# linum-uqam/ViT-OCM-WMSegmentation

Measured on AMD Instinct MI355X. Metric: OCM tiles/s (224x224, ViT-S/16 attention-map inference), higher is better.
Workload: dtype bf16x3

## Files before the change

vit-ocm-wmsegmentation_amd/csrc/engine.hip:

```cpp
#include <stdarg.h>
#include <stdio.h>
#include <string.h>

#include <atomic>
#include <mutex>
#include <string>
#include <vector>

#include "host_common.h"
#include "launch.h"
#include "attn_plan.h"
#include "otsu.h"

static thread_local std::string g_err;

int ocm_fail(int code, const char *fmt, ...) {
    char buf[512];
    va_list ap;
    va_start(ap, fmt);
    vsnprintf(buf, sizeof buf, fmt, ap);
    va_end(ap);
    g_err = buf;
    return code;
}
// ... 272 lines not shown
    void *xn;
    void *q, *k;
    void *vt;
    void *ctx;
    void *hid;
    float *lse;
    float *qkv32;
    float *kpart;
    size_t kpart_bytes;
    float *part;
    float *stats;
    float *shift;
    float *tok_shift;
    size_t bytes;
};

static Workspace carve(const ocm_vit *h, int batch, int n, char *base) {
    Workspace w;
    size_t off = 0;
    auto take = [&](size_t bytes) {
        char *pch = base ? base + off : nullptr;
        off += (bytes + 255) & ~(size_t)255;
        return pch;
    };
    const size_t T = (size_t)batch * n, BH = (size_t)batch * h->H, np = ocm_n_pad_for(h->prec, n);
    const size_t e = h->esz;
    w.x = (float *)take(T * h->D * 4);
    w.xn = take(T * h->D * e);
    w.lse = (float *)take(BH * n * 4);
    w.stats = h->can_fold() ? (float *)take(2 * T * (size_t)(h->D / 64) * 8) : nullptr;
    w.shift = h->can_fold() ? (float *)take(2 * T * 4) : nullptr;
    w.tok_shift = h->can_fold() ? (float *)take((size_t)n * 4) : nullptr;
    w.part = (h->prec == 2 && T <= (size_t)OCM_SPLITK_MAX_ROWS) ? (float *)take((size_t)OCM_SPLITK * T * h->D * 4) : nullptr;
    w.kpart_bytes = attention_ksplit_bytes(h->prec, batch, n, h->H, h->hd);
    w.kpart = w.kpart_bytes ? (float *)take(w.kpart_bytes) : nullptr;
    const size_t base_off = off;
    w.q = w.k = w.vt = nullptr;
    w.qkv32 = nullptr;
    if (h->mfma_heads()) {
        w.q = take(BH * np * h->hd * e);
        w.k = take(BH * np * h->hd * e);
        w.vt = take(BH * np * h->hd * e);
    } else {
        w.qkv32 = (float *)take(3 * T * h->D * 4);
    }
    w.ctx = take(T * h->D * e);
    const size_t attn_end = off;
    off = base_off;
    w.hid = take(T * h->M * e);
    if (off < attn_end) off = attn_end;
    w.bytes = off;
    return w;
}

extern "C" size_t ocm_vit_workspace_bytes(const ocm_vit_t *h, int32_t batch, int32_t n_tokens) {
    if (!h || batch <= 0 || n_tokens <= 1) return 0;
    return carve(h, batch, n_tokens, nullptr).bytes;
}

static int check_ws(const ocm_vit *h, int batch, int n, void *ws, size_t ws_bytes) {
    if (!ws) return fail(OCM_ENOMEM, "workspace is null");
    if ((uintptr_t)ws & 255) return fail(OCM_EINVAL, "workspace must be 256-byte aligned");
    const size_t need = carve(h, batch, n, nullptr).bytes;
    if (ws_bytes < need) return fail(OCM_ENOMEM, "workspace too small: %zu < %zu bytes", ws_bytes, need);
    return OCM_OK;
}

static int run_attention(const ocm_vit *h, const Workspace &w, int batch, int n, bool attn_only, float *out_attn, float *out_qkv,
                         const int32_t *query_rows, int n_rows, float *out_rows, const char *qkv_w, const float *qkv_b,
                         const LnFold &ln, hipStream_t s) {
    const int H = h->H, np = ocm_n_pad_for(h->prec, n), pc = h->prec;
    const float scale = h->cfg.qk_scale;
    const bool want_v = !(attn_only && !out_qkv);
    if (!h->mfma_heads()) {
        float *qkv = out_qkv ? out_qkv : w.qkv32;
        { PROF(OCM_K_QKV, s); HIP_TRY(launch_qkv(pc, w.xn, qkv_w, qkv_b, nullptr, nullptr, nullptr, qkv, batch, n, np, H, h->hd, want_v, s, ln)); }
        { PROF(OCM_K_ATTN, s); HIP_TRY(launch_attention_generic(pc, qkv, attn_only ? nullptr : w.ctx, out_attn, query_rows, n_rows, out_rows, batch, n, H, h->hd, scale, s)); }
        return OCM_OK;
    }
    void *vt_dst = want_v ? w.vt : nullptr;
    { PROF(OCM_K_QKV, s); HIP_TRY(launch_qkv(pc, w.xn, qkv_w, qkv_b, w.q, w.k, vt_dst, out_qkv, batch, n, np, H, h->hd, want_v, s, ln)); }
    if (out_rows && !out_attn) { PROF(OCM_K_PROBS, s); HIP_TRY(launch_attention_rows(pc, w.q, w.k, query_rows, n_rows, out_rows, batch, n, np, H, scale, s, h->hd)); }
    if (attn_only && !out_attn) return OCM_OK;
    { PROF(OCM_K_ATTN, s); HIP_TRY(launch_attention(pc, w.q, w.k, w.vt, attn_only ? nullptr : w.ctx, out_attn ? w.lse : nullptr, batch, n, np, H, scale, s, h->hd, w.kpart, w.kpart_bytes)); }
    if (out_attn) {
        PROF(OCM_K_PROBS, s);
        HIP_TRY(launch_attention_probs(pc, w.q, w.k, w.lse, out_attn, batch, n, np, H, scale, s, h->hd, query_rows, n_rows, out_rows));
    }
    return OCM_OK;
}

static int run_block(const ocm_vit *h, int i, const Workspace &w, float *x, int batch, int n, bool attn_only,
                     float *out_attn, float *out_qkv, const int32_t *query_rows, int n_rows, float *out_rows,
                     hipStream_t s, bool xn_ready = false, const float *next_g = nullptr, const float *next_b = nullptr,
                     bool *xn_out = nullptr) {
    const BlockP &bp = h->blk[i];
    const int D = h->D, T = batch * n;
    const float eps = h->cfg.ln_eps;
    const int pc = h->prec, lnk = ln_kind_of_prec(pc);
    const long t128 = (long)((T + 127) / 128) * (D / 128);
    const int fuse_opt = h->opt[OCM_OPT_FUSE_LN];
    const bool fuse_ln = linear_resid_ln_supported(D) && fuse_opt != 1 && ((T >= 8192 && t128 < 512) || fuse_opt == 2);
    if (xn_out) *xn_out = false;
    if (!xn_ready) { PROF(OCM_K_LN, s); HIP_TRY(launch_layernorm(x, h->ptr<float>(bp.ln1_g), h->ptr<float>(bp.ln1_b), w.xn, lnk, T, D, eps, s)); }
    if (int rc = run_attention(h, w, batch, n, attn_only, out_attn, out_qkv, query_rows, n_rows, out_rows, h->ptr<char>(bp.qkv_w),
                               h->ptr<float>(bp.qkv_b), LnFold(), s))
        return rc;
    if (attn_only) return OCM_OK;
    if (fuse_ln) {
        PROF(OCM_K_PROJ, s);
        HIP_TRY(launch_linear_resid_ln(pc, w.ctx, h->ptr<char>(bp.proj_w), h->ptr<float>(bp.proj_b), x, x, h->ptr<float>(bp.ln2_g), h->ptr<float>(bp.ln2_b), w.xn, T, D, D, eps, s));
    } else {
        { PROF(OCM_K_PROJ, s); HIP_TRY(launch_linear(pc, w.ctx, h->ptr<char>(bp.proj_w), h->ptr<float>(bp.proj_b), x, x, T, D, D, OCM_EPI_BIAS_RESID_F32, s)); }
        { PROF(OCM_K_LN, s); HIP_TRY(launch_layernorm(x, h->ptr<float>(bp.ln2_g), h->ptr<float>(bp.ln2_b), w.xn, lnk, T, D, eps, s)); }
    }
    { PROF(OCM_K_FC1, s); HIP_TRY(launch_linear(pc, w.xn, h->ptr<char>(bp.fc1_w), h->ptr<float>(bp.fc1_b), nullptr, w.hid, T, h->M, D, OCM_EPI_BIAS_GELU_BF16, s)); }
    if (fuse_ln && next_g && next_b) {
        PROF(OCM_K_FC2, s);
        HIP_TRY(launch_linear_resid_ln(pc, w.hid, h->ptr<char>(bp.fc2_w), h->ptr<float>(bp.fc2_b), x, x, next_g, next_b, w.xn, T, D, h->M, eps, s));
        if (xn_out) *xn_out = true;
    } else {
        PROF(OCM_K_FC2, s);
        StatsOut so;
        if (fuse_opt == 0) so.part = w.part;
        HIP_TRY(launch_linear(pc, w.hid, h->ptr<char>(bp.fc2_w), h->ptr<float>(bp.fc2_b), x, x, T, D, h->M, OCM_EPI_BIAS_RESID_F32, s, LnFold(), so));
    }
    return OCM_OK;
}

static int run_block_folded(const ocm_vit *h, int i, const Workspace &w, float *x, int batch, int n, bool attn_only,
                            float *out_attn, float *out_qkv, const int32_t *query_rows, int n_rows, float *out_rows,
                            hipStream_t s) {
    const BlockP &bp = h->blk[i];
    const int D = h->D, T = batch * n, pc = h->prec;
    float *st_in = w.stats, *st_mid = w.stats + (size_t)T * (D / 64) * 2, *st_out = w.stats;
    LnFold ln1, ln2;
    ln1.stats = st_in, ln1.c = h->ptr<float>(bp.qkv_c), ln1.d = h->ptr<float>(bp.qkv_d), ln1.inv_dim = 1.0f / D, ln1.eps = h->cfg.ln_eps;
    ln2.stats = st_mid, ln2.c = h->ptr<float>(bp.fc1_c), ln2.d = h->ptr<float>(bp.fc1_d), ln2.inv_dim = 1.0f / D, ln2.eps = h->cfg.ln_eps;
    ln1.nslot = ln2.nslot = D / 64;
    if (int rc = run_attention(h, w, batch, n, attn_only, out_attn, out_qkv, query_rows, n_rows, out_rows, h->ptr<char>(bp.qkv_wf),
                               nullptr, ln1, s))
        return rc;
    if (attn_only) return OCM_OK;
    StatsOut so_mid, so_out;
    so_mid.xs = w.xn, so_mid.stats = st_mid;
    so_out.xs = w.xn, so_out.stats = st_out;
    float *sh_in = w.shift, *sh_mid = w.shift + T;
    so_mid.shift = sh_mid, so_mid.prev_stats = st_in, so_mid.prev_shift = sh_in;
    so_out.shift = sh_in, so_out.prev_stats = st_mid, so_out.prev_shift = sh_mid;
    so_out.part = w.part;
    { PROF(OCM_K_PROJ, s); HIP_TRY(launch_linear(pc, w.ctx, h->ptr<char>(bp.proj_w), h->ptr<float>(bp.proj_b), x, x, T, D, D, OCM_EPI_BIAS_RESID_F32, s, LnFold(), so_mid)); }
    { PROF(OCM_K_FC1, s); HIP_TRY(launch_linear(pc, w.xn, h->ptr<char>(bp.fc1_wf), nullptr, nullptr, w.hid, T, h->M, D, OCM_EPI_BIAS_GELU_BF16, s, ln2)); }
    { PROF(OCM_K_FC2, s); HIP_TRY(launch_linear(pc, w.hid, h->ptr<char>(bp.fc2_w), h->ptr<float>(bp.fc2_b), x, x, T, D, h->M, OCM_EPI_BIAS_RESID_F32, s, LnFold(), so_out)); }
    return OCM_OK;
}

static int check_tiles(const ocm_vit *h, const ocm_vit_io *io, int *n_out) {
    if (!io) return fail(OCM_EINVAL, "io is null");
    if (!io->image) return fail(OCM_EINVAL, "io->image is null");
    if (!io->pos_embed) return fail(OCM_EINVAL, "io->pos_embed is null");
    if (io->batch <= 0) return fail(OCM_EINVAL, "batch %d must be positive", io->batch);
    if (io->tile_h <= 0 || io->tile_w <= 0 || io->tile_h % h->p || io->tile_w % h->p)
        return fail(OCM_EINVAL, "tile %dx%d must be a positive multiple of patch_size %d", io->tile_h, io->tile_w, h->p);
    if (io->img_stride_y % 4 || ((uintptr_t)io->image & 15) || io->img_stride_c % 4 || io->img_stride_b % 4)
        return fail(OCM_EINVAL, "image base must be 16-byte aligned and strides multiples of 4 elements");
    *n_out = (io->tile_h / h->p) * (io->tile_w / h->p) + 1;
    return OCM_OK;
}

static int run_prepare(const ocm_vit *h, const ocm_vit_io *io, float *x, int n, hipStream_t s, void *xs = nullptr,
// ... 256 lines not shown

extern "C" int ocm_op_linear_resid_ln(int32_t precision, const void *a, const void *w, const float *bias,
                                      const float *resid, float *x, const float *gamma, const float *beta, void *xn,
                                      int32_t M, int32_t D, int32_t K, float eps, void *stream) {
    int pc = 0, rc = prec_of(precision, &pc);
    if (rc) return rc;
    if (!a || !w || !resid || !x || !gamma || !beta || !xn) return fail(OCM_EINVAL, "null argument");
    if (!linear_resid_ln_supported(D)) return fail(OCM_EINVAL, "row width %d not in {128, 256, 384}", D);
    if (M <= 0 || K <= 0 || K % 64) return fail(OCM_EINVAL, "bad shape M=%d K=%d (K%%64)", M, K);
    HIP_TRY(launch_linear_resid_ln(pc, a, w, bias, resid, x, gamma, beta, xn, M, D, K, eps, (hipStream_t)stream));
    return OCM_OK;
}

static int op_qkv_proj(int32_t precision, const void *a, const void *w, const float *bias, void *q, void *k, void *vt,
                       float *qkv_f32, int32_t batch, int32_t n_tokens, int32_t heads, int32_t head_dim, void *stream) {
    int pc = 0, rc = prec_of(precision, &pc);
    if (rc) return rc;
    const bool copies = q || k || vt;
    if (!a || !w || !bias || (copies && (!q || !k || !vt)) || (!copies && !qkv_f32)) return fail(OCM_EINVAL, "null argument");
    if (batch <= 0 || n_tokens <= 0 || heads <= 0 || head_dim <= 0 || head_dim % 8) return fail(OCM_EINVAL, "bad shape");
    if ((heads * head_dim) % 64)
        return fail(OCM_EINVAL, "heads * head_dim = %d must be a multiple of 64", heads * head_dim);
    if (copies && head_dim != 64 && head_dim != 128)
        return fail(OCM_EINVAL, "head_dim %d: operand copies exist for 64- and 128-wide heads", head_dim);
    HIP_TRY(launch_qkv(pc, a, w, bias, q, k, vt, qkv_f32, batch, n_tokens, ocm_n_pad_for(pc, n_tokens), heads, head_dim, true,
                       (hipStream_t)stream));
    return OCM_OK;
}

extern "C" int ocm_op_qkv_proj(int32_t precision, const void *a, const void *w, const float *bias, void *q, void *k,
                               void *vt, float *qkv_f32, int32_t batch, int32_t n_tokens, int32_t heads, void *stream) {
    return op_qkv_proj(precision, a, w, bias, q, k, vt, qkv_f32, batch, n_tokens, heads, 64, stream);
}

extern "C" int ocm_op_qkv_proj_hd(int32_t precision, const void *a, const void *w, const float *bias, void *q, void *k,
                                  void *vt, float *qkv_f32, int32_t batch, int32_t n_tokens, int32_t heads,
                                  int32_t head_dim, void *stream) {
    return op_qkv_proj(precision, a, w, bias, q, k, vt, qkv_f32, batch, n_tokens, heads, head_dim, stream);
}

static int attention_shape_ok(int32_t batch, int32_t n_tokens, int32_t heads, int32_t head_dim) {
    if (batch <= 0 || n_tokens <= 0 || heads <= 0) return fail(OCM_EINVAL, "bad shape");
    if (head_dim != 64 && head_dim != 128)
        return fail(OCM_EINVAL, "head_dim %d: the MFMA attention is built for 64- and 128-wide heads", head_dim);
    return OCM_OK;
}

static int op_attention(int32_t precision, const void *q, const void *k, const void *vt, void *ctx, float *lse2,
                        int32_t batch, int32_t n_tokens, int32_t heads, int32_t head_dim, float scale, void *stream,
                        void *workspace = nullptr, size_t workspace_bytes = 0) {
    int pc = 0, rc = prec_of(precision, &pc);
    if (rc) return rc;
    if (!q || !k || !vt || (!ctx && !lse2)) return fail(OCM_EINVAL, "null argument");
    if ((rc = attention_shape_ok(batch, n_tokens, heads, head_dim))) return rc;
    if (workspace && (uintptr_t)workspace % 16) return fail(OCM_EINVAL, "workspace must be 16-byte aligned");
    HIP_TRY(launch_attention(pc, q, k, vt, ctx, lse2, batch, n_tokens, ocm_n_pad_for(pc, n_tokens), heads, scale,
                             (hipStream_t)stream, head_dim, (float *)workspace, workspace ? workspace_bytes : 0));
    return OCM_OK;
}

extern "C" int ocm_attention_plan(int32_t precision, int32_t batch, int32_t n_tokens, int32_t heads, int32_t head_dim,
                                  size_t workspace_bytes, ocm_attention_plan_info *plan) {
    int pc = 0, rc = prec_of(precision, &pc);
    if (rc) return rc;
    if (!plan) return fail(OCM_EINVAL, "null argument");
    if ((rc = attention_shape_ok(batch, n_tokens, heads, head_dim))) return rc;
    const AttnPlan p = attn_plan(pc, batch, n_tokens, heads, head_dim, workspace_bytes);
    *plan = ocm_attention_plan_info{(int32_t)p.kernel, p.waves, p.stages, p.kslices, (int32_t)p.grid_x, (int32_t)p.grid_y,
                                    (int32_t)p.grid_z, p.lds_bytes, (uint64_t)p.workspace_need};
    return OCM_OK;
}

extern "C" size_t ocm_attention_workspace_bytes(int32_t precision, int32_t batch, int32_t n_tokens, int32_t heads,
                                                int32_t head_dim) {
    int pc = 0;
    if (prec_of(precision, &pc) || attention_shape_ok(batch, n_tokens, heads, head_dim)) return 0;
    return attention_ksplit_bytes(pc, batch, n_tokens, heads, head_dim);
}

static int op_attention_probs(int32_t precision, const void *q, const void *k, const float *lse2, float *attn, int32_t batch,
                              int32_t n_tokens, int32_t heads, int32_t head_dim, float scale, void *stream) {
    int pc = 0, rc = prec_of(precision, &pc);
    if (rc) return rc;
    if (!q || !k || !lse2 || !attn) return fail(OCM_EINVAL, "null argument");
    if (batch <= 0 || n_tokens <= 0 || heads <= 0) return fail(OCM_EINVAL, "bad shape");
    if (head_dim != 64 && head_dim != 128) return fail(OCM_EINVAL, "head_dim %d not built on MFMA", head_dim);
    HIP_TRY(launch_attention_probs(pc, q, k, lse2, attn, batch, n_tokens, ocm_n_pad_for(pc, n_tokens), heads, scale,
                                   (hipStream_t)stream, head_dim));
    return OCM_OK;
}

extern "C" int ocm_op_attention(int32_t precision, const void *q, const void *k, const void *vt, void *ctx, float *lse2,
                                int32_t batch, int32_t n_tokens, int32_t heads, float scale, void *stream) {
    return op_attention(precision, q, k, vt, ctx, lse2, batch, n_tokens, heads, 64, scale, stream);
}

extern "C" int ocm_op_attention_hd(int32_t precision, const void *q, const void *k, const void *vt, void *ctx, float *lse2,
                                   int32_t batch, int32_t n_tokens, int32_t heads, int32_t head_dim, float scale,
                                   void *stream) {
    return op_attention(precision, q, k, vt, ctx, lse2, batch, n_tokens, heads, head_dim, scale, stream);
}

extern "C" int ocm_op_attention_ws(int32_t precision, const void *q, const void *k, const void *vt, void *ctx, float *lse2,
                                   int32_t batch, int32_t n_tokens, int32_t heads, int32_t head_dim, float scale,
                                   void *workspace, size_t workspace_bytes, void *stream) {
    return op_attention(precision, q, k, vt, ctx, lse2, batch, n_tokens, heads, head_dim, scale, stream, workspace, workspace_bytes);
}

extern "C" int ocm_op_attention_generic(int32_t precision, const float *qkv_f32, void *ctx, float *attn, int32_t batch,
                                        int32_t n_tokens, int32_t heads, int32_t head_dim, float scale, void *stream) {
    int pc = 0, rc = prec_of(precision, &pc);
    if (rc) return rc;
    if (!qkv_f32 || (!ctx && !attn)) return fail(OCM_EINVAL, "null argument");
    if (batch <= 0 || n_tokens <= 0 || heads <= 0 || head_dim <= 0) return fail(OCM_EINVAL, "bad shape");
    if (head_dim % 4 || head_dim > 512 || n_tokens > 8192 || (pc == 2 && (heads * head_dim) % 32))
        return fail(OCM_EINVAL, "generic attention: head_dim %d must be a multiple of 4 up to 512, at most 8192 tokens, and "
                                "heads * head_dim a multiple of 32 for a split-bf16 context", head_dim);
    if ((int64_t)batch * heads > 65535) return fail(OCM_EINVAL, "batch * heads = %lld > 65535", (long long)batch * heads);
    HIP_TRY(launch_attention_generic(pc, qkv_f32, ctx, attn, nullptr, 0, nullptr, batch, n_tokens, heads, head_dim, scale,
                                     (hipStream_t)stream));
    return OCM_OK;
}

extern "C" int ocm_op_attention_probs(int32_t precision, const void *q, const void *k, const float *lse2, float *attn,
                                      int32_t batch, int32_t n_tokens, int32_t heads, float scale, void *stream) {
    return op_attention_probs(precision, q, k, lse2, attn, batch, n_tokens, heads, 64, scale, stream);
}

extern "C" int ocm_op_attention_probs_hd(int32_t precision, const void *q, const void *k, const float *lse2, float *attn,
                                         int32_t batch, int32_t n_tokens, int32_t heads, int32_t head_dim, float scale,
                                         void *stream) {
    return op_attention_probs(precision, q, k, lse2, attn, batch, n_tokens, heads, head_dim, scale, stream);
}

extern "C" int ocm_op_attention_rows(int32_t precision, const void *q, const void *k, const int32_t *query_rows,
                                     int32_t n_rows, float *rows, int32_t batch, int32_t n_tokens, int32_t heads,
                                     float scale, void *stream) {
    int pc = 0, rc = prec_of(precision, &pc);
    if (rc) return rc;
    if (!q || !k || !rows) return fail(OCM_EINVAL, "null argument");
    if (batch <= 0 || n_tokens <= 1 || heads <= 0 || n_rows <= 0) return fail(OCM_EINVAL, "bad shape");
    HIP_TRY(launch_attention_rows(pc, q, k, query_rows, n_rows, rows, batch, n_tokens, ocm_n_pad_for(pc, n_tokens), heads, scale,
                                  (hipStream_t)stream));
    return OCM_OK;
}

extern "C" int ocm_op_attention_map(const float *attn, float *maps, int32_t b, int32_t heads, int32_t n_tokens,
                                    int32_t query, int32_t hf, int32_t wf, int32_t p, void *stream) {
    if (!attn || !maps) return fail(OCM_EINVAL, "null argument");
    if (hf * wf + 1 != n_tokens) return fail(OCM_EINVAL, "hf*wf+1 = %d != n_tokens %d", hf * wf + 1, n_tokens);
    if (query < 0 || query >= n_tokens) return fail(OCM_EINVAL, "query %d out of range", query);
    HIP_TRY(launch_attention_map(attn, maps, b, heads, n_tokens, query, hf, wf, p, (hipStream_t)stream));
    return OCM_OK;
}

extern "C" int ocm_op_tile_postprocess(const float *rows, float *maps, int32_t tiles, int32_t heads, int32_t n_rows,
                                       int32_t pixels, void *stream) {
    if (!rows || !maps) return fail(OCM_EINVAL, "null argument");
    if (tiles <= 0 || heads <= 0 || n_rows <= 0 || pixels <= 0) return fail(OCM_EINVAL, "bad shape");
    HIP_TRY(launch_tile_postprocess(rows, maps, tiles, heads, n_rows, pixels, (hipStream_t)stream));
    return OCM_OK;
}

extern "C" int ocm_op_bilinear_upsample(const float *src, float *dst, int32_t tiles, int32_t h, int32_t w,
                                        int32_t scale, void *stream) {
    if (!src || !dst) return fail(OCM_EINVAL, "null argument");
    if (tiles <= 0 || h <= 0 || w <= 0 || scale <= 0) return fail(OCM_EINVAL, "bad shape");
    HIP_TRY(launch_bilinear_up(src, dst, tiles, h, w, scale, (hipStream_t)stream));
    return OCM_OK;
// ... 160 lines not shown
```

vit-ocm-wmsegmentation_amd/csrc/kernels_attn.hip:

```cpp
#include <stdlib.h>

#include "launch.h"

#define LOG2E 1.4426950408889634f
#include "attn_plan.h"
#define OCM_VMCNT_ATTN(n) asm volatile("s_waitcnt vmcnt(%0)" ::"n"(n) : "memory")

#ifndef OCM_DEFER_MAX
#define OCM_DEFER_MAX 8.0f
#endif
__device__ __forceinline__ float defer_max_update(float &m, float cand) {
    if (__any(cand > m + OCM_DEFER_MAX)) {
        const float mn = fmaxf(m, cand);
        const float alpha = fast_exp2(m - mn);
        m = mn;
        return alpha;
    }
    return 1.0f;
}

template <bool WANT_O, int HD = 64>
__global__ __launch_bounds__(256, HD == 64 ? 3 : 2) void attn_fwd_kernel(const bf16 *__restrict__ Q, const bf16 *__restrict__ Kk,
                                                       const bf16 *__restrict__ Vt, bf16 *__restrict__ ctx,
                                                       float *__restrict__ lse2, int N, int npad, int H,
// ... 1146 lines not shown
    const int c = (threadIdx.x % LPR) * 4;
    const int64_t stride = (int64_t)BH * N * (HD + 4);
    const float *p = part + row * (HD + 4);
    float m = -INFINITY;
    for (int s = 0; s < nslice; ++s) m = fmaxf(m, p[s * stride + HD]);
    float L = 0.f;
    f32x4 o = {0.f, 0.f, 0.f, 0.f};
    for (int s = 0; s < nslice; ++s) {
        const f32x2 ml = *(const f32x2 *)(p + s * stride + HD);
        const float wgt = fast_exp2(ml[0] - m);
        L = fmaf(ml[1], wgt, L);
        if (ctx) o += *(const f32x4 *)(p + s * stride + c) * wgt;
    }
    if (ctx) {
        const float inv = 1.0f / L;
        const int bh = (int)(row / N), q = (int)(row - (int64_t)bh * N), b = bh / H, head = bh - b * H;
        bf16x4 hi, lo;
        split4(o * inv, hi, lo);
        char *dst = ctx + ((int64_t)b * N + q) * (H * HD) * 4 + head * (HD * 4) + sp_off(c);
        *(bf16x4 *)dst = hi;
        *(bf16x4 *)(dst + 64) = lo;
    }
    if (lse2 && c == 0) lse2[row] = m + __log2f(L);
}

template <int HD>
__global__ __launch_bounds__(256) void attn_probs_x3_kernel(const char *__restrict__ Q, const char *__restrict__ Kk,
                                                            const float *__restrict__ lse2, float *__restrict__ attn,
                                                            int N, int npad, float scale2) {
    const int lane = threadIdx.x & 63, wave = threadIdx.x >> 6;
    const int r = lane & 31, h = lane >> 5;
    int qblk, bh;
    xcd_remap2(qblk, bh);
    const int q0 = (qblk * 4 + wave) * 32;
    if (q0 >= N) return;
    constexpr int NQ = HD / 16;
    const char *Qb = Q + (int64_t)bh * npad * (HD * 4);
    const char *Kb = Kk + (int64_t)bh * npad * (HD * 4);
    auto loadrow = [&](const char *base, int row, bf16x8(&hi)[NQ], bf16x8(&lo)[NQ]) {
        const char *rp = base + (int64_t)row * (HD * 4);
#pragma unroll
        for (int s = 0; s < NQ; ++s) {
            const char *p = rp + (s >> 1) * 128 + ((s & 1) * 16 + 8 * h) * 2;
            hi[s] = *(const bf16x8 *)p;
            lo[s] = *(const bf16x8 *)(p + 64);
        }
    };
    bf16x8 qh[NQ], ql[NQ];
    loadrow(Qb, min(q0 + r, N - 1), qh, ql);
    float lr[16];
#pragma unroll
    for (int e = 0; e < 16; ++e) lr[e] = lse2[(int64_t)bh * N + min(q0 + acc_row32(e, h), N - 1)];
    float *out = attn + (int64_t)bh * N * N;
    const int nkt = (N + 31) >> 5, per = (nkt + (int)gridDim.z - 1) / (int)gridDim.z;
    const int kt0 = (int)blockIdx.z * per, ktiles = min(nkt, kt0 + per);
    if (kt0 >= ktiles) return;
    bf16x8 kh[NQ], kl[NQ], nh[NQ], nl[NQ];
    loadrow(Kb, min(kt0 * 32 + r, N - 1), kh, kl);
    for (int kt = kt0; kt < ktiles; ++kt) {
        if (kt + 1 < ktiles) loadrow(Kb, min((kt + 1) * 32 + r, N - 1), nh, nl);
        f32x16 S;
#pragma unroll
        for (int e = 0; e < 16; ++e) S[e] = 0.f;
#pragma unroll
        for (int s = 0; s < NQ; ++s) S = mfma32x3(qh[s], ql[s], kh[s], kl[s], S);
        const int key = kt * 32 + r;
        if (key < N) {
#pragma unroll
            for (int e = 0; e < 16; ++e) {
                const int qrow = q0 + acc_row32(e, h);
                if (qrow < N) out[(int64_t)qrow * N + key] = fast_exp2(S[e] * scale2 - lr[e]);
            }
        }
#pragma unroll
        for (int s = 0; s < NQ; ++s) {
            kh[s] = nh[s];
            kl[s] = nl[s];
        }
    }
}

constexpr int PROBS_FOLD_ROWS = 8;

__global__ __launch_bounds__(256) void attn_probs_x3_span_kernel(const char *__restrict__ Q, const char *__restrict__ Kk,
                                                                 const float *__restrict__ lse2, float *__restrict__ attn,
                                                                 int N, int npad, float scale2,
                                                                 const int32_t *__restrict__ query_rows, int n_rows,
                                                                 float *__restrict__ rows) {
    constexpr int HD = 64, NQ = HD / 16, ROWB = HD * 4, PITCH = ROWB + 16, REGION = 32 * PITCH, TILEB = 32 * ROWB;
    __shared__ __attribute__((aligned(16))) char smem[4 * REGION];
    const int tid = threadIdx.x, lane = tid & 63, wave = tid >> 6;
    const int r = lane & 31, h = lane >> 5;
    int qblk, bh;
    xcd_remap2(qblk, bh);
    const int q0 = qblk * 32, nq = min(32, N - q0);
    const int nkt = (N + 31) >> 5;
    const char *Qb = Q + ((int64_t)bh * npad + q0) * ROWB;
    const char *Kb = Kk + (int64_t)bh * npad * ROWB;
    f32x4 qraw[2], kraw[2][8];
#pragma unroll
    for (int i = 0; i < 2; ++i) qraw[i] = *(const f32x4 *)(Qb + (i * 256 + tid) * 16);
#pragma unroll
    for (int t = 0; t < 2; ++t)
        if (wave + 4 * t < nkt) {
#pragma unroll
            for (int i = 0; i < 8; ++i) kraw[t][i] = *(const f32x4 *)(Kb + (int64_t)(wave + 4 * t) * TILEB + (i * 64 + lane) * 16);
        }
    float lr[16];
#pragma unroll
    for (int e = 0; e < 16; ++e) lr[e] = lse2[(int64_t)bh * N + min(q0 + acc_row32(e, h), N - 1)];
    auto stage = [&](char *region, int piece, const f32x4 &v) {
        *(f32x4 *)(region + (piece >> 4) * PITCH + (piece & 15) * 16) = v;
    };
    auto fragments = [&](const char *region, bf16x8(&hi)[NQ], bf16x8(&lo)[NQ]) {
        const char *rp = region + r * PITCH;
#pragma unroll
        for (int s = 0; s < NQ; ++s) {
            const char *p = rp + (s >> 1) * 128 + ((s & 1) * 16 + 8 * h) * 2;
            hi[s] = *(const bf16x8 *)p;
            lo[s] = *(const bf16x8 *)(p + 64);
        }
    };
    bf16x8 qh[NQ], ql[NQ];
#pragma unroll
    for (int i = 0; i < 2; ++i) stage(smem, i * 256 + tid, qraw[i]);
    lds_barrier();
    fragments(smem, qh, ql);
    lds_barrier();
    char *mine = smem + wave * REGION;
    float pr[2][16];
#pragma unroll
    for (int t = 0; t < 2; ++t) {
        const bool have = wave + 4 * t < nkt;
        if (have) {
#pragma unroll
            for (int i = 0; i < 8; ++i) stage(mine, i * 64 + lane, kraw[t][i]);
        }
        lds_barrier();
        if (have) {
            bf16x8 kh[NQ], kl[NQ];
            fragments(mine, kh, kl);
            f32x16 S;
#pragma unroll
            for (int e = 0; e < 16; ++e) S[e] = 0.f;
#pragma unroll
            for (int s = 0; s < NQ; ++s) S = mfma32x3(qh[s], ql[s], kh[s], kl[s], S);
#pragma unroll
            for (int e = 0; e < 16; ++e) pr[t][e] = fast_exp2(S[e] * scale2 - lr[e]);
        }
        lds_barrier();
    }
    float *span = attn + ((int64_t)bh * N + q0) * N;
    const int shift = (int)(((uintptr_t)span >> 2) & 3);
    float *img = (float *)smem + shift;
#pragma unroll
    for (int t = 0; t < 2; ++t) {
        const int key = (wave + 4 * t) * 32 + r;
        if (key < N) {
#pragma unroll
            for (int e = 0; e < 16; ++e) {
                const int row = acc_row32(e, h);
                if (row < nq) img[row * N + key] = pr[t][e];
            }
        }
    }
    lds_barrier();
    const int len = nq * N;
    const int lead = min((4 - shift) & 3, len), nvec = (len - lead) >> 2, tail = lead + 4 * nvec;
    if (tid < lead) span[tid] = img[tid];
    for (int i = tid; i < nvec; i += 256) *(f32x4 *)(span + lead + 4 * i) = *(const f32x4 *)(img + lead + 4 * i);
    if (tid < len - tail) span[tail + tid] = img[tail + tid];
    if (rows) {
        for (int i = 0; i < n_rows; ++i) {
            const int query = query_rows ? query_rows[i] : 0;
            if (query < q0 || query >= q0 + nq) continue;
            float *dst = rows + ((int64_t)bh * n_rows + i) * (N - 1);
            const float *src = img + (query - q0) * N + 1;
            for (int j = tid; j < N - 1; j += 256) dst[j] = src[j];
        }
    }
}


__device__ __forceinline__ void store_ctx1(int prec, char *rowp, int col, float v) {
    if (prec == 0) {
        *(bf16 *)(rowp + col * 2) = (bf16)v;
    } else if (prec == 1) {
        *(float *)(rowp + col * 4) = v;
    } else {
        bf16 hi, lo;
        split1(v, hi, lo);
        *(bf16 *)(rowp + sp_off(col)) = hi;
        *(bf16 *)(rowp + sp_off(col) + 64) = lo;
    }
}

__global__ __launch_bounds__(256) void attn_generic_kernel(const float *__restrict__ qkv, char *__restrict__ ctx,
                                                           float *__restrict__ attn, const int32_t *__restrict__ query_rows,
                                                           int n_rows, float *__restrict__ rows, int B, int H, int N,
                                                           int hd, float scale, int prec, bool all_queries) {
    extern __shared__ __attribute__((aligned(16))) char smem[];
    const int lane = threadIdx.x & 63, wave = threadIdx.x >> 6;
    float *qs = (float *)smem + wave * (hd + N);
    float *sc = qs + hd;
    const int bh = blockIdx.y, b = bh / H, head = bh - b * H;
    const int qi = blockIdx.x * 4 + wave;
    const int nq = all_queries ? N : n_rows;
    if (qi >= nq) return;
    const int query = all_queries ? qi : (query_rows ? query_rows[qi] : 0);
    const size_t plane = (size_t)B * H * N * hd;
    const float *Q = qkv + ((size_t)bh * N + query) * hd;
    const float *K = qkv + plane + (size_t)bh * N * hd;
    const float *V = qkv + 2 * plane + (size_t)bh * N * hd;
    for (int d = lane; d < hd; d += 64) qs[d] = Q[d];
    __builtin_amdgcn_wave_barrier();
    float mx = -INFINITY;
    for (int key = lane; key < N; key += 64) {
        const float *kp = K + (size_t)key * hd;
        float acc = 0.f;
        for (int d = 0; d < hd; d += 4) {
            const f32x4 kv = *(const f32x4 *)(kp + d), qv = *(const f32x4 *)(qs + d);
            acc = fmaf(qv[0], kv[0], acc);
            acc = fmaf(qv[1], kv[1], acc);
            acc = fmaf(qv[2], kv[2], acc);
            acc = fmaf(qv[3], kv[3], acc);
        }
        acc *= scale;
        sc[key] = acc;
        mx = fmaxf(mx, acc);
    }
#pragma unroll
    for (int o = 32; o > 0; o >>= 1) mx = fmaxf(mx, __shfl_xor(mx, o, 64));
    float sum = 0.f;
    for (int key = lane; key < N; key += 64) {
        const float p = __expf(sc[key] - mx);
        sc[key] = p;
        sum += p;
    }
#pragma unroll
    for (int o = 32; o > 0; o >>= 1) sum += __shfl_xor(sum, o, 64);
    const float inv = 1.0f / sum;
    for (int key = lane; key < N; key += 64) sc[key] *= inv;
    __builtin_amdgcn_wave_barrier();
    if (attn && all_queries) {
        float *dst = attn + ((size_t)bh * N + query) * N;
// ... 47 lines not shown

hipError_t launch_attention(int prec, const void *q, const void *k, const void *vt, void *ctx, float *lse2, int batch,
                            int n_tokens, int n_pad, int heads, float scale, hipStream_t s, int head_dim, float *ksplit_ws,
                            size_t ksplit_bytes) {
    if (head_dim != 64 && head_dim != 128) return hipErrorInvalidValue;
    if (prec == 2 && n_pad % 32) return hipErrorInvalidValue;
    const AttnPlan p = attn_plan(prec, batch, n_tokens, heads, head_dim, ksplit_ws ? ksplit_bytes : 0);
    const dim3 grid(p.grid_x, p.grid_y, p.grid_z), block(p.waves * 64);
    const float scale2 = scale * LOG2E;
    const char *Q = (const char *)q, *K = (const char *)k, *V = (const char *)vt;
    switch (p.kernel) {
        case ATTN_BF16_WHOLE: {
            auto kern = ctx ? attn_small_kernel<true> : attn_small_kernel<false>;
            kern<<<grid, block, 0, s>>>((const bf16 *)q, (const bf16 *)k, (const bf16 *)vt, (bf16 *)ctx, lse2, n_tokens, n_pad, heads,
                                        scale2);
            break;
        }
        case ATTN_BF16_STREAM: {
            auto kern = head_dim == 128 ? (ctx ? attn_fwd_kernel<true, 128> : attn_fwd_kernel<false, 128>)
                                        : (ctx ? attn_fwd_kernel<true> : attn_fwd_kernel<false>);
            kern<<<grid, block, 0, s>>>((const bf16 *)q, (const bf16 *)k, (const bf16 *)vt, (bf16 *)ctx, lse2, n_tokens, n_pad, heads,
                                        scale2);
            break;
        }
        case ATTN_F32_STREAM: {
            auto kern = head_dim == 128 ? (ctx ? attn_fwd_f32_kernel<true, 128> : attn_fwd_f32_kernel<false, 128>)
                                        : (ctx ? attn_fwd_f32_kernel<true> : attn_fwd_f32_kernel<false>);
            if (p.lds_bytes > 64 * 1024) {
                static OptinMask optin[2];
                if (hipError_t e = lds_optin((const void *)kern, p.lds_bytes, optin[ctx ? 1 : 0]); e != hipSuccess) return e;
            }
            kern<<<grid, block, p.lds_bytes, s>>>((const float *)q, (const float *)k, (const float *)vt, (float *)ctx, lse2, n_tokens,
                                                  n_pad, heads, scale2);
            break;
        }
        case ATTN_X3_WS: {
            auto kern = ctx ? attn_fwd_x3_ws_kernel<true> : attn_fwd_x3_ws_kernel<false>;
            static OptinMask optin[2];
            if (hipError_t e = lds_optin((const void *)kern, p.lds_bytes, optin[ctx ? 1 : 0]); e != hipSuccess) return e;
            kern<<<grid, block, p.lds_bytes, s>>>(Q, K, V, (char *)ctx, lse2, n_tokens, n_pad, heads, scale2);
            break;
        }
        case ATTN_X3_PP: {
            auto kern = ctx ? attn_fwd_x3_pp_kernel<true> : attn_fwd_x3_pp_kernel<false>;
            kern<<<grid, block, 0, s>>>(Q, K, V, (char *)ctx, lse2, n_tokens, n_pad, heads, scale2);
            break;
        }
        case ATTN_X3_DMA:
            if (head_dim == 128) {
                auto kern = ctx ? attn_fwd_x3_dma_kernel<true, 4, 2, 128, 2> : attn_fwd_x3_dma_kernel<false, 4, 2, 128, 2>;
                kern<<<grid, block, 0, s>>>(Q, K, V, (char *)ctx, lse2, n_tokens, n_pad, heads, scale2, 0, nullptr);
            } else {
                auto kern = ctx ? attn_fwd_x3_dma_kernel<true, 8, 2> : attn_fwd_x3_dma_kernel<false, 8, 2>;
                kern<<<grid, block, 0, s>>>(Q, K, V, (char *)ctx, lse2, n_tokens, n_pad, heads, scale2, (OCM_WT_MASK >> 4) & 1,
                                            nullptr);
            }
            break;
        case ATTN_X3_DMA_KSPLIT: {
            auto kern = ctx ? attn_fwd_x3_dma_kernel<true, 8, 2, 64, 3, true> : attn_fwd_x3_dma_kernel<false, 8, 2, 64, 3, true>;
            kern<<<grid, block, 0, s>>>(Q, K, V, (char *)ctx, lse2, n_tokens, n_pad, heads, scale2, 0, ksplit_ws);
            if (hipError_t e = hipGetLastError(); e != hipSuccess) return e;
            const int64_t rows = (int64_t)batch * heads * n_tokens;
            attn_merge_x3_kernel<64><<<dim3((unsigned)((rows + 15) / 16)), dim3(256), 0, s>>>(
                ksplit_ws, p.kslices, (char *)ctx, lse2, batch * heads, n_tokens, heads);
            break;
        }
    }
    return hipGetLastError();
}

template <int HD>
static hipError_t launch_probs_hd(int prec, const void *q, const void *k, const float *lse2, float *attn, int n_tokens, int n_pad,
                                  float scale2, dim3 grid, dim3 gridz, hipStream_t s) {
    const dim3 block(256);
    if (prec == 2)
        attn_probs_x3_kernel<HD><<<gridz, block, 0, s>>>((const char *)q, (const char *)k, lse2, attn, n_tokens, n_pad, scale2);
    else if (prec)
        attn_probs_f32_kernel<HD><<<grid, block, 0, s>>>((const float *)q, (const float *)k, lse2, attn, n_tokens, n_pad, scale2);
    else
        attn_probs_kernel<HD><<<grid, block, 0, s>>>((const bf16 *)q, (const bf16 *)k, lse2, attn, n_tokens, n_pad, scale2);
    return hipGetLastError();
}

hipError_t launch_attention_probs(int prec, const void *q, const void *k, const float *lse2, float *attn, int batch,
                                  int n_tokens, int n_pad, int heads, float scale, hipStream_t s, int head_dim,
                                  const int32_t *query_rows, int n_rows, float *rows) {
    if (head_dim != 64 && head_dim != 128) return hipErrorInvalidValue;
    const int qtiles = (n_tokens + 31) / 32;
    const dim3 grid((qtiles + 3) / 4, batch * heads);
    const int wgs = (int)(grid.x * grid.y), ktiles = qtiles;
    const int nz = wgs >= 256 ? 1 : min(ktiles, min(16, (512 + wgs - 1) / wgs));
    const dim3 gridz(grid.x, grid.y, nz);
    if (n_rows <= 0) rows = nullptr;
    bool folded = false;
    hipError_t e;
    if (prec == 2 && head_dim == 64 && n_tokens <= 255 && n_pad % 32 == 0 && n_pad >= n_tokens) {
        folded = rows && n_rows <= PROBS_FOLD_ROWS;
        attn_probs_x3_span_kernel<<<dim3(qtiles, batch * heads), dim3(256), 0, s>>>(
            (const char *)q, (const char *)k, lse2, attn, n_tokens, n_pad, scale * LOG2E, query_rows, n_rows, folded ? rows : nullptr);
        e = hipGetLastError();
    } else if (head_dim == 128) {
        e = launch_probs_hd<128>(prec, q, k, lse2, attn, n_tokens, n_pad, scale * LOG2E, grid, gridz, s);
    } else {
        e = launch_probs_hd<64>(prec, q, k, lse2, attn, n_tokens, n_pad, scale * LOG2E, grid, gridz, s);
    }
    if (e != hipSuccess || !rows || folded) return e;
    return launch_rows_from_probs(attn, query_rows, n_rows, rows, batch, n_tokens, heads, s);
}

__device__ __forceinline__ void load8(const bf16 *rowp, int c, float (&o)[8]) {
    const bf16x8 t = *(const bf16x8 *)(rowp + c * 8);
#pragma unroll
    for (int e = 0; e < 8; ++e) o[e] = (float)t[e];
}
__device__ __forceinline__ void load8(const float *rowp, int c, float (&o)[8]) {
    const f32x4 a = *(const f32x4 *)(rowp + c * 8), b = *(const f32x4 *)(rowp + c * 8 + 4);
#pragma unroll
    for (int e = 0; e < 4; ++e) {
        o[e] = a[e];
        o[4 + e] = b[e];
    }
}
__device__ __forceinline__ void load8(const sp32 *rowp, int c, float (&o)[8]) {
    const char *p = (const char *)rowp + sp_off(c * 8);
    const bf16x8 hi = *(const bf16x8 *)p, lo = *(const bf16x8 *)(p + 64);
#pragma unroll
    for (int e = 0; e < 8; ++e) o[e] = (float)hi[e] + (float)lo[e];
}

template <class E, int HD>
__global__ __launch_bounds__(64) void attn_rows_kernel(const E *__restrict__ Q, const E *__restrict__ Kk,
                                                       const int32_t *__restrict__ query_rows, int n_rows,
                                                       float *__restrict__ rows, int N, int npad, float scale2) {
    extern __shared__ __attribute__((aligned(16))) char smem[];
    float *sc = (float *)smem;
    const int lane = threadIdx.x, bh = blockIdx.y, qi = blockIdx.x;
    const int query = query_rows ? query_rows[qi] : 0;
    const E *qp = Q + ((int64_t)bh * npad + query) * HD;
    float qv[HD];
#pragma unroll
    for (int c = 0; c < HD / 8; ++c) {
        float t[8];
        load8(qp, c, t);
#pragma unroll
        for (int e = 0; e < 8; ++e) qv[c * 8 + e] = t[e];
    }
    float mx = -INFINITY;
    for (int key = lane; key < N; key += 64) {
        const E *kp = Kk + ((int64_t)bh * npad + key) * HD;
        float acc = 0.f;
#pragma unroll
        for (int c = 0; c < HD / 8; ++c) {
            float t[8];
            load8(kp, c, t);
#pragma unroll
            for (int e = 0; e < 8; ++e) acc = fmaf(qv[c * 8 + e], t[e], acc);
        }
        acc *= scale2;
        sc[key] = acc;
        mx = fmaxf(mx, acc);
    }
#pragma unroll
    for (int o = 32; o > 0; o >>= 1) mx = fmaxf(mx, __shfl_xor(mx, o, 64));
    float sum = 0.f;
    for (int key = lane; key < N; key += 64) {
        const float p = fast_exp2(sc[key] - mx);
        sc[key] = p;
        sum += p;
    }
#pragma unroll
    for (int o = 32; o > 0; o >>= 1) sum += __shfl_xor(sum, o, 64);
    const float inv = 1.0f / sum;
    float *dst = rows + ((int64_t)bh * n_rows + qi) * (N - 1);
    for (int key = 1 + lane; key < N; key += 64) dst[key - 1] = sc[key] * inv;
}

__global__ __launch_bounds__(256) void rows_from_probs_kernel(const float *__restrict__ attn,
                                                              const int32_t *__restrict__ query_rows, int n_rows,
                                                              float *__restrict__ rows, int N, size_t total) {
    for (size_t i = (size_t)blockIdx.x * 256 + threadIdx.x; i < total; i += (size_t)gridDim.x * 256) {
        const int j = (int)(i % (N - 1));
        const size_t t = i / (N - 1);
        const int qi = (int)(t % n_rows);
// ... 66 lines not shown
```

vit-ocm-wmsegmentation_amd/csrc/launch.h:

```cpp
#pragma once
#include <atomic>
#include "common.h"
#include "gemm_plan.h"

typedef std::atomic<unsigned long long> OptinMask;
static inline hipError_t lds_optin(const void *kern, int bytes, OptinMask &done) {
    int dev = 0;
    if (hipError_t e = hipGetDevice(&dev); e != hipSuccess) return e;
    const unsigned long long bit = 1ull << (dev & 63);
    if (done.load(std::memory_order_acquire) & bit) return hipSuccess;
    const hipError_t e = hipFuncSetAttribute(kern, hipFuncAttributeMaxDynamicSharedMemorySize, bytes);
    if (e == hipSuccess) done.fetch_or(bit, std::memory_order_release);
    return e;
}

constexpr int OCM_WT_MASK = 35;

hipError_t launch_layernorm(const float *x, const float *gamma, const float *beta, void *y, int out_kind,
                            int64_t rows, int dim, float eps, hipStream_t s);
static inline int ln_kind_of_prec(int prec) { return prec == 0 ? 1 : prec == 1 ? 0 : 2; }
hipError_t launch_cast_bf16(const float *src, bf16 *dst, size_t count, hipStream_t s);
hipError_t launch_cast_split(const float *src, void *dst, size_t count, hipStream_t s);
hipError_t launch_merge_split(const void *src, float *dst, size_t count, hipStream_t s);
hipError_t launch_fold_split(const float *src, void *dst, int D, int C, int pp, hipStream_t s);
hipError_t launch_fold_cast_bf16(const float *src, bf16 *dst, int D, int C, int pp, hipStream_t s);
hipError_t launch_fold_f32(const float *src, float *dst, int D, int C, int pp, hipStream_t s);
hipError_t launch_im2col3x3(int prec, const float *in, void *out, int batch, int h, int w, int C, int relu, hipStream_t s);
hipError_t launch_bn_relu_im2col3x3(int prec, const float *in, const float *scale, const float *shift, void *out, int batch,
                                    int h, int w, int C, hipStream_t s);
hipError_t launch_cls_rows(const float *cls, const float *pos, float *x, int batch, int n_tokens, int dim,
                           hipStream_t s);
struct LnFold {
    const float *stats = nullptr;
    const float *c = nullptr, *d = nullptr;
    float inv_dim = 0.f, eps = 0.f;
    int nslot = 0;
};
struct StatsOut {
    void *xs = nullptr;
    float *stats = nullptr;
    float *shift = nullptr;
    const float *prev_stats = nullptr, *prev_shift = nullptr;
    const float *tok_shift = nullptr;
    float *part = nullptr;
};
hipError_t launch_splitk_finish(const float *part, int slices, const float *bias, const float *resid, float *x, void *xs,
                                float *stats, int M, int N, hipStream_t s, const StatsOut &so = StatsOut());
hipError_t launch_cls_rows_stats(const float *cls, const float *pos, float *x, void *xs, float *stats, int batch,
                                 int n_tokens, int dim, hipStream_t s, float *shift = nullptr, float *tok_shift = nullptr,
                                 const float *pe_bias = nullptr);
hipError_t launch_fold_ln(const float *W, const float *gamma, const float *beta, const float *bias, void *Wf, float *cvec,
                          float *dvec, int N, int K, hipStream_t s);

hipError_t launch_linear(int prec, const void *a, const void *w, const float *bias, const float *resid, void *out, int M,
                         int N, int K, int epilogue, hipStream_t s, const LnFold &ln = LnFold(),
                         const StatsOut &so = StatsOut());
bool linear_resid_ln_supported(int D);
hipError_t launch_linear_resid_ln(int prec, const void *a, const void *w, const float *bias, const float *resid, float *x,
                                  const float *gamma, const float *beta, void *xn, int M, int D, int K, float eps,
                                  hipStream_t s);
hipError_t launch_qkv(int prec, const void *a, const void *w, const float *bias, void *q, void *k, void *vt,
                      float *qkv_f32, int batch, int n_tokens, int n_pad, int heads, int head_dim, bool want_v,
                      hipStream_t s, const LnFold &ln = LnFold());
hipError_t launch_attention_generic(int prec, const float *qkv, void *ctx, float *attn, const int32_t *query_rows,
                                    int n_rows, float *rows, int batch, int n_tokens, int heads, int head_dim, float scale,
                                    hipStream_t s);
struct PatchArgs {
    const float *image;
    int64_t sb, sc, sy;
    const int32_t *origins;
    int batch, hp, wp, p, chans;
    const float *mask = nullptr;
    const float *mask_tok = nullptr;
};
hipError_t launch_patch_embed(int prec, const PatchArgs &pa, const void *w, const float *bias, const float *pos,
                              float *x, int dim, hipStream_t s, const StatsOut &so = StatsOut());

hipError_t launch_attention(int prec, const void *q, const void *k, const void *vt, void *ctx, float *lse2, int batch,
                            int n_tokens, int n_pad, int heads, float scale, hipStream_t s, int head_dim = 64,
                            float *ksplit_ws = nullptr, size_t ksplit_bytes = 0);
size_t attention_ksplit_bytes(int prec, int batch, int n_tokens, int heads, int head_dim);
hipError_t launch_attention_probs(int prec, const void *q, const void *k, const float *lse2, float *attn, int batch,
                                  int n_tokens, int n_pad, int heads, float scale, hipStream_t s, int head_dim = 64,
                                  const int32_t *query_rows = nullptr, int n_rows = 0, float *rows = nullptr);
hipError_t launch_rows_from_probs(const float *attn, const int32_t *query_rows, int n_rows, float *rows, int batch,
                                  int n_tokens, int heads, hipStream_t s);
hipError_t launch_attention_rows(int prec, const void *q, const void *k, const int32_t *query_rows, int n_rows,
                                 float *rows, int batch, int n_tokens, int n_pad, int heads, float scale, hipStream_t s,
                                 int head_dim = 64);
hipError_t launch_attention_map(const float *attn, float *maps, int b, int heads, int n_tokens, int query, int hf,
                                int wf, int p, hipStream_t s);

hipError_t launch_tile_postprocess(const float *rows, float *maps, int tiles, int heads, int n_rows, int pixels,
                                   hipStream_t s);
hipError_t launch_bilinear_up(const float *src, float *dst, int tiles, int h, int w, int scale, hipStream_t s);
hipError_t launch_nearest_up(const float *src, float *dst, int tiles, int h, int w, int rep, hipStream_t s);
hipError_t launch_stitch(const float *crops, float *out, const double *ramp, int n, int window, int stride,
                         hipStream_t s);
hipError_t launch_normalize_u8(const float *img, size_t count, float *part, uint8_t *out,
                               unsigned long long *hist256, hipStream_t s);
hipError_t launch_threshold_u8(const uint8_t *img, uint8_t *mask, size_t count, int thresh, hipStream_t s);
hipError_t launch_tokens_to_fmap(const float *y, float *out, int batch, int n_tokens, int dim, hipStream_t s);
hipError_t launch_pixel_shuffle(const float *lin, float *out, int batch, int hp, int wp, int c_out, int sh, hipStream_t s);
hipError_t launch_head_mean(const float *rows, float *maps, int tiles, int heads, int n_rows, int pixels, hipStream_t s);
hipError_t launch_image_to_gray_u8(const float *img, int64_t stride_c, int chans, size_t count, uint8_t *out,
                                   unsigned long long *hist256, hipStream_t s);
hipError_t launch_blend_u8(const uint8_t *img, const uint8_t *att, size_t count, double alpha, double one_minus_alpha,
                           uint8_t *out, unsigned long long *hist256, hipStream_t s);

hipError_t launch_stitch_image_u8(const float *image, int64_t sc, int64_t sy, int chans, int H, int W, uint8_t *out,
                                  const double *ramp, int n, int window, int stride, unsigned long long *hist256,
                                  hipStream_t s);
hipError_t launch_weighted_u8(const float *heat, const uint8_t *img, size_t count, float *part, uint8_t *result,
                              uint8_t *att_u8, unsigned long long *hist_res, unsigned long long *hist_att, hipStream_t s);
hipError_t launch_histogram_u8(const uint8_t *img, size_t count, unsigned long long *hist256, hipStream_t s);
hipError_t launch_median_filter(const float *src, float *dst, int tiles, int h, int w, int k, hipStream_t s);
hipError_t launch_downscale_centre(const float *src, float *dst, int tiles, int h, int w, int f, hipStream_t s);

static inline int ocm_round_up(int v, int m) { return (v + m - 1) / m * m; }
static inline int ocm_n_pad_for(int prec, int n) { return ocm_round_up(n, prec == 2 ? 32 : 8); }

hipError_t launch_linear_ld(int prec, const void *a, int64_t lda, const void *w, const float *bias, const float *resid,
                            void *out, int64_t ldo, int M, int N, int K, int epilogue, hipStream_t s);
hipError_t launch_swin_embed(const float *img, const float *w, const float *bias, const float *g, const float *be,
                             float *x, int batch, int chans, int size, int c0, float eps, hipStream_t s);
hipError_t launch_swin_ln(int prec, const float *x, const float *g, const float *be, void *y, size_t rows, int dim,
                          int ldy, float eps, bool merge, int Hin, int Win, hipStream_t s);
hipError_t launch_swin_pad_rows(const void *src, void *dst, int batch, int H, int W, int Hp, int Wp, size_t row_bytes,
                                hipStream_t s);
hipError_t launch_swin_crop_add(float *x, const float *yp, int batch, int H, int W, int Hp, int Wp, int C, hipStream_t s);
constexpr int OCM_SWIN_WIDE_BINS = 544;
static inline size_t swin_bias_floats(int ws, int heads) {
    return ws > 7 ? (size_t)heads * OCM_SWIN_WIDE_BINS : (size_t)heads * (4096 + (size_t)ws * ws * ws * ws);
}
hipError_t launch_swin_bias_perm(const float *table, float *perm, float *dense, int heads, int ws, hipStream_t s);
hipError_t launch_swin_window_attention(int prec, const void *qkv, int ld, void *ctx, int ldc, const float *bias_perm,
                                        const float *bias_dense, int batch, int H, int W, int ws, int shift, int heads,
                                        hipStream_t s);
hipError_t launch_swin_window_probs(int prec, const void *qkv, int ld, float *probs, const float *bias_perm,
                                    const float *bias_dense, int batch, int H, int W, int ws, int shift, int heads, hipStream_t s);
hipError_t launch_swin_tokens_to_nchw(const float *x, float *out, int batch, int L, int C, hipStream_t s);
bool swin_lnqkv_fused_supported(int prec, int C);
hipError_t launch_swin_lnqkv(int prec, const float *x, const float *g, const float *be, const void *w, const float *bias,
                             void *qkv, size_t T, int C, float eps, hipStream_t s);
hipError_t launch_swin_lnlinear(int prec, const float *x, const float *g, const float *be, const void *w, const float *bias,
                                void *out, size_t T, int C, int N, bool gelu, float eps, hipStream_t s);
bool swin_mlp_fused_supported(int prec, int C, int hidden);
hipError_t launch_swin_mlp(int prec, float *x, const float *g, const float *be, const void *w1, const float *b1,
                           const void *w2, const float *b2, size_t T, int C, int hidden, float eps, hipStream_t s);
bool swin_attn_block_fused_supported(int prec, int C, int heads, int ws);
bool swin_attn_block_proj_fused(int C);
hipError_t launch_swin_attn_block(int prec, float *x, const float *g, const float *be, const void *wqkv, const float *bqkv,
                                  const void *wo, const float *bo, const float *bias_perm, void *ctx, int batch, int H, int W,
                                  int ws, int shift, int heads, int C, float eps, hipStream_t s);
hipError_t launch_swin_pool_head(const float *x, const float *g, const float *be, const float *cw, const float *cb,
                                 float *logits, float *pooled, float *hidden, int batch, int L, int C, int labels,
                                 float eps, hipStream_t s);
hipError_t launch_swin_mask_tokens(float *rows, const uint8_t *mask, const float *token, size_t tokens, int channels,
                                   hipStream_t s);
hipError_t launch_cast_pad(int prec, const float *src, void *dst, size_t rows, int K, int Kp, hipStream_t s);
```

Before: 27710.

## Compute softmax stats inside span probs kernel, skip attention pass when attn-only

For split-bf16, 64-wide heads and up to 255 tokens, the attention-probability span kernel now computes row max and sum itself with a cross-wave LDS reduction instead of reading log-sum-exp from the flash attention kernel. When only attention maps are needed, the full attention forward launch is skipped entirely. This removes a whole kernel pass over Q/K/V, at the cost of a transposed MFMA layout and extra barriers in the probs kernel.

Result: no change. 27850 (median of 6 runs) (+0.5%).

```diff
diff --git a/vit-ocm-wmsegmentation_amd/csrc/engine.hip b/vit-ocm-wmsegmentation_amd/csrc/engine.hip
--- a/vit-ocm-wmsegmentation_amd/csrc/engine.hip
+++ b/vit-ocm-wmsegmentation_amd/csrc/engine.hip
@@ -378,10 +378,12 @@
     { PROF(OCM_K_QKV, s); HIP_TRY(launch_qkv(pc, w.xn, qkv_w, qkv_b, w.q, w.k, vt_dst, out_qkv, batch, n, np, H, h->hd, want_v, s, ln)); }
     if (out_rows && !out_attn) { PROF(OCM_K_PROBS, s); HIP_TRY(launch_attention_rows(pc, w.q, w.k, query_rows, n_rows, out_rows, batch, n, np, H, scale, s, h->hd)); }
     if (attn_only && !out_attn) return OCM_OK;
-    { PROF(OCM_K_ATTN, s); HIP_TRY(launch_attention(pc, w.q, w.k, w.vt, attn_only ? nullptr : w.ctx, out_attn ? w.lse : nullptr, batch, n, np, H, scale, s, h->hd, w.kpart, w.kpart_bytes)); }
+    const bool own_stats = out_attn && attention_probs_span_serves(pc, n, np, h->hd);
+    float *lse = out_attn && !own_stats ? w.lse : nullptr;
+    if (!attn_only || lse) { PROF(OCM_K_ATTN, s); HIP_TRY(launch_attention(pc, w.q, w.k, w.vt, attn_only ? nullptr : w.ctx, lse, batch, n, np, H, scale, s, h->hd, w.kpart, w.kpart_bytes)); }
     if (out_attn) {
         PROF(OCM_K_PROBS, s);
-        HIP_TRY(launch_attention_probs(pc, w.q, w.k, w.lse, out_attn, batch, n, np, H, scale, s, h->hd, query_rows, n_rows, out_rows));
+        HIP_TRY(launch_attention_probs(pc, w.q, w.k, lse, out_attn, batch, n, np, H, scale, s, h->hd, query_rows, n_rows, out_rows));
     }
     return OCM_OK;
 }
@@ -804,9 +806,11 @@
                               int32_t n_tokens, int32_t heads, int32_t head_dim, float scale, void *stream) {
     int pc = 0, rc = prec_of(precision, &pc);
     if (rc) return rc;
-    if (!q || !k || !lse2 || !attn) return fail(OCM_EINVAL, "null argument");
+    if (!q || !k || !attn) return fail(OCM_EINVAL, "null argument");
     if (batch <= 0 || n_tokens <= 0 || heads <= 0) return fail(OCM_EINVAL, "bad shape");
     if (head_dim != 64 && head_dim != 128) return fail(OCM_EINVAL, "head_dim %d not built on MFMA", head_dim);
+    if (!lse2 && !attention_probs_span_serves(pc, n_tokens, ocm_n_pad_for(pc, n_tokens), head_dim))
+        return fail(OCM_EINVAL, "a null lse2 needs split-bf16, 64-wide heads and at most 255 tokens");
     HIP_TRY(launch_attention_probs(pc, q, k, lse2, attn, batch, n_tokens, ocm_n_pad_for(pc, n_tokens), heads, scale,
                                    (hipStream_t)stream, head_dim));
     return OCM_OK;
diff --git a/vit-ocm-wmsegmentation_amd/csrc/kernels_attn.hip b/vit-ocm-wmsegmentation_amd/csrc/kernels_attn.hip
--- a/vit-ocm-wmsegmentation_amd/csrc/kernels_attn.hip
+++ b/vit-ocm-wmsegmentation_amd/csrc/kernels_attn.hip
@@ -1252,6 +1252,7 @@
 
 constexpr int PROBS_FOLD_ROWS = 8;
 
+template <bool OWN>
 __global__ __launch_bounds__(256) void attn_probs_x3_span_kernel(const char *__restrict__ Q, const char *__restrict__ Kk,
                                                                  const float *__restrict__ lse2, float *__restrict__ attn,
                                                                  int N, int npad, float scale2,
@@ -1277,8 +1278,10 @@
             for (int i = 0; i < 8; ++i) kraw[t][i] = *(const f32x4 *)(Kb + (int64_t)(wave + 4 * t) * TILEB + (i * 64 + lane) * 16);
         }
     float lr[16];
-#pragma unroll
-    for (int e = 0; e < 16; ++e) lr[e] = lse2[(int64_t)bh * N + min(q0 + acc_row32(e, h), N - 1)];
+    if constexpr (!OWN) {
+#pragma unroll
+        for (int e = 0; e < 16; ++e) lr[e] = lse2[(int64_t)bh * N + min(q0 + acc_row32(e, h), N - 1)];
+    }
     auto stage = [&](char *region, int piece, const f32x4 &v) {
         *(f32x4 *)(region + (piece >> 4) * PITCH + (piece & 15) * 16) = v;
     };
@@ -1299,6 +1302,7 @@
     lds_barrier();
     char *mine = smem + wave * REGION;
     float pr[2][16];
+    float wmax = -INFINITY;
 #pragma unroll
     for (int t = 0; t < 2; ++t) {
         const bool have = wave + 4 * t < nkt;
@@ -1313,24 +1317,66 @@
             f32x16 S;
 #pragma unroll
             for (int e = 0; e < 16; ++e) S[e] = 0.f;
-#pragma unroll
-            for (int s = 0; s < NQ; ++s) S = mfma32x3(qh[s], ql[s], kh[s], kl[s], S);
-#pragma unroll
-            for (int e = 0; e < 16; ++e) pr[t][e] = fast_exp2(S[e] * scale2 - lr[e]);
+            if constexpr (OWN) {
+#pragma unroll
+                for (int s = 0; s < NQ; ++s) S = mfma32x3(kh[s], kl[s], qh[s], ql[s], S);
+#pragma unroll
+                for (int e = 0; e < 16; ++e) {
+                    pr[t][e] = S[e] * scale2;
+                    if ((wave + 4 * t) * 32 + acc_row32(e, h) < N) wmax = fmaxf(wmax, pr[t][e]);
+                }
+            } else {
+#pragma unroll
+                for (int s = 0; s < NQ; ++s) S = mfma32x3(qh[s], ql[s], kh[s], kl[s], S);
+#pragma unroll
+                for (int e = 0; e < 16; ++e) pr[t][e] = fast_exp2(S[e] * scale2 - lr[e]);
+            }
         }
         lds_barrier();
     }
     float *span = attn + ((int64_t)bh * N + q0) * N;
     const int shift = (int)(((uintptr_t)span >> 2) & 3);
     float *img = (float *)smem + shift;
-#pragma unroll
-    for (int t = 0; t < 2; ++t) {
-        const int key = (wave + 4 * t) * 32 + r;
-        if (key < N) {
-#pragma unroll
-            for (int e = 0; e < 16; ++e) {
-                const int row = acc_row32(e, h);
-                if (row < nq) img[row * N + key] = pr[t][e];
+    if constexpr (OWN) {
+        __shared__ float stat[2][4][32];
+        wmax = fmaxf(wmax, __shfl_xor(wmax, 32));
+        if (h == 0) stat[0][wave][r] = wmax;
+        lds_barrier();
+        const float m = fmaxf(fmaxf(stat[0][0][r], stat[0][1][r]), fmaxf(stat[0][2][r], stat[0][3][r]));
+        float wsum = 0.f;
+#pragma unroll
+        for (int t = 0; t < 2; ++t)
+            if (wave + 4 * t < nkt) {
+#pragma unroll
+                for (int e = 0; e < 16; ++e) {
+                    const bool valid = (wave + 4 * t) * 32 + acc_row32(e, h) < N;
+                    pr[t][e] = valid ? fast_exp2(pr[t][e] - m) : 0.f;
+                    wsum += pr[t][e];
+                }
+            }
+        wsum += __shfl_xor(wsum, 32);
+        if (h == 0) stat[1][wave][r] = wsum;
+        lds_barrier();
+        const float inv = 1.0f / ((stat[1][0][r] + stat[1][1][r]) + (stat[1][2][r] + stat[1][3][r]));
+        if (r < nq) {
+#pragma unroll
+            for (int t = 0; t < 2; ++t)
+#pragma unroll
+                for (int e = 0; e < 16; ++e) {
+                    const int key = (wave + 4 * t) * 32 + acc_row32(e, h);
+                    if (key < N) img[r * N + key] = pr[t][e] * inv;
+                }
+        }
+    } else {
+#pragma unroll
+        for (int t = 0; t < 2; ++t) {
+            const int key = (wave + 4 * t) * 32 + r;
+            if (key < N) {
+#pragma unroll
+                for (int e = 0; e < 16; ++e) {
+                    const int row = acc_row32(e, h);
+                    if (row < nq) img[row * N + key] = pr[t][e];
+                }
             }
         }
     }
@@ -1544,6 +1590,10 @@
     return hipGetLastError();
 }
 
+bool attention_probs_span_serves(int prec, int n_tokens, int n_pad, int head_dim) {
+    return prec == 2 && head_dim == 64 && n_tokens <= 255 && n_pad % 32 == 0 && n_pad >= n_tokens;
+}
+
 hipError_t launch_attention_probs(int prec, const void *q, const void *k, const float *lse2, float *attn, int batch,
                                   int n_tokens, int n_pad, int heads, float scale, hipStream_t s, int head_dim,
                                   const int32_t *query_rows, int n_rows, float *rows) {
@@ -1556,11 +1606,14 @@
     if (n_rows <= 0) rows = nullptr;
     bool folded = false;
     hipError_t e;
-    if (prec == 2 && head_dim == 64 && n_tokens <= 255 && n_pad % 32 == 0 && n_pad >= n_tokens) {
+    if (attention_probs_span_serves(prec, n_tokens, n_pad, head_dim)) {
         folded = rows && n_rows <= PROBS_FOLD_ROWS;
-        attn_probs_x3_span_kernel<<<dim3(qtiles, batch * heads), dim3(256), 0, s>>>(
+        auto kern = lse2 ? attn_probs_x3_span_kernel<false> : attn_probs_x3_span_kernel<true>;
+        kern<<<dim3(qtiles, batch * heads), dim3(256), 0, s>>>(
             (const char *)q, (const char *)k, lse2, attn, n_tokens, n_pad, scale * LOG2E, query_rows, n_rows, folded ? rows : nullptr);
         e = hipGetLastError();
+    } else if (!lse2) {
+        return hipErrorInvalidValue;
     } else if (head_dim == 128) {
         e = launch_probs_hd<128>(prec, q, k, lse2, attn, n_tokens, n_pad, scale * LOG2E, grid, gridz, s);
     } else {
diff --git a/vit-ocm-wmsegmentation_amd/csrc/launch.h b/vit-ocm-wmsegmentation_amd/csrc/launch.h
--- a/vit-ocm-wmsegmentation_amd/csrc/launch.h
+++ b/vit-ocm-wmsegmentation_amd/csrc/launch.h
@@ -80,6 +80,7 @@
                             int n_tokens, int n_pad, int heads, float scale, hipStream_t s, int head_dim = 64,
                             float *ksplit_ws = nullptr, size_t ksplit_bytes = 0);
 size_t attention_ksplit_bytes(int prec, int batch, int n_tokens, int heads, int head_dim);
+bool attention_probs_span_serves(int prec, int n_tokens, int n_pad, int head_dim);
 hipError_t launch_attention_probs(int prec, const void *q, const void *k, const float *lse2, float *attn, int batch,
                                   int n_tokens, int n_pad, int heads, float scale, hipStream_t s, int head_dim = 64,
                                   const int32_t *query_rows = nullptr, int n_rows = 0, float *rows = nullptr);
```
